# Rick0514/SimpleSLAM

Measured on AMD Instinct MI355X. Metric: scans/s (65 k-pt scan vs 1 M-pt submap, LOAM 10 iters) + pose RMSE vs CPU ref, higher is better.
Workload: dtype f64; 1 GPU; pcr=loam, 65536-pt 64-beam scan vs 1000000-pt submap, 10 GN iters, early exit off, index rebuilt per call (previous call's bounding box and tile layout reused as checked hints), inputs in HBM; parallelism=single GPU, scans_cycled=8

## Files before the change

### include/pcr_hip.h

```cpp
#ifndef PCR_HIP_H
#define PCR_HIP_H

#include <stddef.h>
#include <stdint.h>

#ifdef __cplusplus
extern "C" {
#endif

typedef struct pcr_handle pcr_handle;

typedef struct pcr_params {
    uint32_t struct_size;
    int32_t device;

    int32_t loam_iters;
    int32_t loam_early_exit;
    double loam_knn_max_sq;
    double loam_plane_thresh;
    double loam_point_thresh;
    double loam_pos_conv;
    double loam_rot_conv;

    double ndt_resolution;
// ... 19 lines not shown
    int32_t record_timeline;
    int32_t loam_coresident;
    int32_t loam_clamp_margin_mm;
    int32_t full_target;
    int32_t host_optimiser;
    int32_t host_copy_xyz;
} pcr_params;

typedef struct pcr_stats {
    double total_ms;
    double index_ms;
    double solve_ms;
    double kernel_ms;
    int32_t kernel_launches;
    int32_t iterations;
    int64_t n_src, n_dst;
    int32_t attempts;
    int32_t target_builds;
    int32_t region_repeats;
    int32_t region_index;
    double aux_kernel_ms;
    int64_t region_points, region_voxels, pairs_grad, pairs_hess;
    int32_t index_box_hint, index_layout_hint;
} pcr_stats;

void pcr_default_params(pcr_params* p);

pcr_handle* pcr_create(const char* method, const pcr_params* p);
void pcr_destroy(pcr_handle* h);
const char* pcr_last_error(const pcr_handle* h);

int pcr_scan2map(pcr_handle* h, const void* src, size_t n_src, const void* dst, size_t n_dst,
                 size_t stride_bytes, double pose_inout[16], int* converged);

int pcr_host_pin(const void* ptr, size_t bytes);
int pcr_host_unpin(const void* ptr);

int pcr_scan2map_device(pcr_handle* h, const void* d_src, size_t n_src, const void* d_dst, size_t n_dst,
                        size_t stride_bytes, double pose_inout[16], int* converged);

int pcr_set_target(pcr_handle* h, const void* dst, size_t n_dst, size_t stride_bytes, int on_device);
int pcr_align(pcr_handle* h, const void* src, size_t n_src, size_t stride_bytes, int on_device,
              double pose_inout[16], int* converged);
int pcr_invalidate_target(pcr_handle* h);

double pcr_fitness(pcr_handle* h);
// ... 166 lines not shown
```

### simpleslam_amd/csrc/capi.hip

```cpp
#include <dlfcn.h>
#include <math.h>
#include <string.h>

#include <algorithm>
#include <atomic>
#include <functional>
#include <mutex>
#include <vector>

#include "pcr_internal.h"
#include "ndt_opt.h"
#include "vgicp_opt.h"
#include "small_math.h"

using namespace pcr;

namespace {

thread_local std::string g_create_error;

enum Method { kLoam = 0, kNdt = 1, kVgicp = 2 };

struct NcclId { char internal[128]; };
typedef int (*nccl_get_id_fn)(NcclId*);
// ... 286 lines not shown
    a->c.knn_max_sq = h->prm.loam_knn_max_sq; a->c.plane_thresh = h->prm.loam_plane_thresh;
    a->c.point_thresh = h->prm.loam_point_thresh; a->c.pos_conv = h->prm.loam_pos_conv; a->c.rot_conv = h->prm.loam_rot_conv;
    a->c.iters = h->prm.loam_iters; a->c.early_exit = h->prm.loam_early_exit;
    memcpy(a->init_pose, pose, 16 * sizeof(double));
    a->state = h->loam_state.as<LoamState>();
    a->partials = h->loam_partials.as<double>();
    a->reduced = nullptr;
    a->n_partials = loam_grid_blocks((uint32_t)n_src);
    h->last_blocks = a->n_partials;
    a->trace = h->prm.record_trace ? h->loam_trace.as<LoamTrace>() : nullptr;
    a->result = h->result.dev;
    a->coresident = h->prm.loam_coresident == 1;
    if (h->prm.loam_disable_cache == 0 && h->nn_cache.reserve((n_src + 1) * 192) == hipSuccess) a->nn_cache = (NnCacheEntry*)h->nn_cache.p;
    if (h->prm.record_timeline == 1 && h->timeline.reserve((size_t)(std::max(1, h->prm.loam_iters) + 1) * kMaxPartials * kTimelineSlots * sizeof(unsigned long long)) == hipSuccess)
        a->timeline = h->timeline.as<unsigned long long>();
    a->use_tile = h->use_tile;
    for (int d = 0; d < 3; ++d) { a->tile_lo[d] = h->tile_lo[d]; a->tile_hi[d] = h->tile_hi[d]; }
}

int build_target(pcr_handle* h, const float* d_dst, size_t n_dst, size_t stride_floats) {
    double cell = 1.0;
    if (h->method == kLoam) cell = grid_cell_for(h->prm.loam_knn_max_sq);
    h->grid.no_hints = h->prm.index_no_hints != 0;
    hipError_t e = h->grid.build(d_dst, n_dst, stride_floats, cell, h->stream, &h->err, 0.0, 0, h->clamp.use ? &h->clamp : nullptr, h->method == kLoam);
    if (e != hipSuccess) return 1;
    h->tgt_ptr = d_dst; h->tgt_n = n_dst; h->tgt_stride = stride_floats; h->have_target = true;
    return 0;
}

static constexpr double kClampMargin = 10.0;
static constexpr int kClampRetries = 6;

int set_clamp_from_scan(pcr_handle* h, const float* d_src, size_t n_src, size_t stride_floats, const double pose[16]) {
    if (!n_src) return fail(h, "target bounding box too large for the dense index and the scan is empty");
    if (h->src_grid.build(d_src, n_src, stride_floats, 1.0, h->stream, &h->err) != hipSuccess) return 1;
    GridHeader sh;
    H_TRY(hipMemcpyAsync(&sh, h->src_grid.header.p, sizeof sh, hipMemcpyDeviceToHost, h->stream));
    H_TRY(hipStreamSynchronize(h->stream));
    if (sh.empty) return fail(h, "target bounding box too large for the dense index and the scan has no finite point");
    double lo[3], hi[3], mlo[3] = {1e300, 1e300, 1e300}, mhi[3] = {-1e300, -1e300, -1e300};
    for (int d = 0; d < 3; ++d) { lo[d] = sh.origin[d]; hi[d] = sh.origin[d] + sh.dims[d] * sh.cell; }
    for (int c = 0; c < 8; ++c) {
        const double p[3] = {c & 1 ? hi[0] : lo[0], c & 2 ? hi[1] : lo[1], c & 4 ? hi[2] : lo[2]};
        for (int r = 0; r < 3; ++r) {
            const double v = pose[r] * p[0] + pose[4 + r] * p[1] + pose[8 + r] * p[2] + pose[12 + r];
            mlo[r] = std::min(mlo[r], v); mhi[r] = std::max(mhi[r], v);
        }
// ... 32 lines not shown
    if (!overflow) return 0;
    if (need_cells > 4000000000ull && h->method == kLoam && d_src && pose && !h->clamp.use) {
        if (set_clamp_from_scan(h, d_src, n_src, stride_floats, pose)) return 1;
        if (build_target(h, h->tgt_ptr, h->tgt_n, h->tgt_stride)) return 1;
        return 2;
    }
    if (need_cells > 4000000000ull && h->method == kLoam && h->clamp_from_bulk && !h->clamp.use) {
        if (set_clamp_from_target_sample(h)) return 1;
        if (build_target(h, h->tgt_ptr, h->tgt_n, h->tgt_stride)) return 1;
        return 2;
    }
    if (h->grid.grow_cells(need_cells, &h->err) != hipSuccess) return 1;
    if (build_target(h, h->tgt_ptr, h->tgt_n, h->tgt_stride)) return 1;
    return 2;
}

int settle_loam_index(pcr_handle* h, const float* d_src, size_t n_src, size_t stride_floats, const double* pose) {
    for (int attempt = 0; attempt < 6; ++attempt) {
        GridHeader hdr;
        H_TRY(hipMemcpyAsync(&hdr, h->grid.header.p, sizeof(hdr), hipMemcpyDeviceToHost, h->stream));
        H_TRY(hipStreamSynchronize(h->stream));
        if (hdr.stale) {
            h->grid.hint_margin = 8; h->grid.cells_hint = 0;
            if (build_target(h, h->tgt_ptr, h->tgt_n, h->tgt_stride)) return 1;
            continue;
        }
        const int ov = check_grid_overflow(h, hdr.overflow, hdr.n_cells, h->clamp_allowed ? d_src : nullptr, n_src, stride_floats, pose);
        if (ov == 0) { if (!hdr.empty) { h->grid.confirm(); h->grid.note_cells(hdr.n_cells); } return 0; }
        if (ov == 1) return 1;
    }
    return fail(h, "target index could not be sized");
}

int run_loam(pcr_handle* h, const float* d_src, size_t n_src, size_t stride_floats, double pose[16], int* converged,
             bool index_timed) {
    if (n_src > 0xfffffff0ull) return fail(h, "source cloud too large");
    if (peer_check(h)) return 1;
    if (ensure_loam_buffers(h)) return 1;
    const int iters = std::max(0, h->prm.loam_iters);
    const bool shard = sharded(h);
    h->clamp_margin = h->prm.loam_clamp_margin_mm != 0 ? 1e-3 * h->prm.loam_clamp_margin_mm : kClampMargin;
    const double margin_cap = kClampMargin * (1 << kClampRetries);
    for (int attempt = 0; attempt < 24; ++attempt) {
        bool rank_fail = false;
        std::string rank_err;
        if (shard) {
// ... 57 lines not shown
            volatile int32_t* flag = &h->result.host->pad;
            for (int spin = 0; spin < 200000 && *flag != 1; ++spin) __builtin_ia32_pause();
            std::atomic_thread_fence(std::memory_order_acquire);
            if (*flag != 1) H_TRY(hipStreamSynchronize(h->stream));
        } else {
            H_TRY(hipStreamSynchronize(h->stream));
        }
        const LoamResult r = *h->result.host;
        if (r.pad != 1) return fail(h, "LOAM finalize kernel did not complete");
        if (peer_check(h)) return 1;
        if (r.fail == 2 || rank_fail)
            return fail(h, rank_fail ? "this rank could not index its map tile: " + rank_err : "sharded scan2map: another rank could not index its map tile");
        if (r.fail == 3) {
            h->clamp_margin = std::max(2.0 * h->clamp_margin, h->clamp_margin + 1.0);
            if (h->clamp_margin > margin_cap) return fail(h, "the pose left the region of a target too sparse for the dense index (a stray point far from the map?)");
            if (h->clamp.use) {
                if (set_clamp_from_scan(h, d_src, n_src, stride_floats, pose)) { if (!shard) return 1; h->grid.valid = false; }
                else if (build_target(h, h->tgt_ptr, h->tgt_n, h->tgt_stride)) { if (!shard) return 1; }
            }
            index_timed = false;
            continue;
        }
        if (!shard) {
            if (r.grid_stale) {
                h->grid.hint_margin = 8; h->grid.cells_hint = 0;
                if (build_target(h, h->tgt_ptr, h->tgt_n, h->tgt_stride)) return 1;
                index_timed = false;
                continue;
            }
            int ov = check_grid_overflow(h, r.grid_overflow, r.grid_cells, h->clamp_allowed ? d_src : nullptr, n_src, stride_floats, pose);
            if (ov == 1) return 1;
            if (ov == 2) { index_timed = false; continue; }
            if (!h->clamp.use && !r.grid_empty) { h->grid.confirm(); h->grid.note_cells(r.grid_cells); }
        }
        memcpy(pose, r.pose, 16 * sizeof(double));
        if (converged) *converged = r.converged;
        h->stats.iterations = r.iters_run; h->stats.attempts = attempt + 1;
        h->stats.n_src = (int64_t)n_src; h->stats.n_dst = (int64_t)h->tgt_n;
        h->stats.kernel_ms = 0; h->stats.kernel_launches = 0;
        if (h->profile >= 1 && read_call_times(h)) return 1;
        if (per_kernel) {
            const int used = std::min(iters, r.converged || r.fail ? r.iters_run : iters);
            for (int k = 0; k < used; ++k) {
                float ms = 0;
                H_TRY(hipEventElapsedTime(&ms, h->ev_kernel[2 * k], h->ev_kernel[2 * k + 1]));
                h->stats.kernel_ms += ms; h->stats.kernel_launches++;
// ... 1524 lines not shown

int pcr_get_timeline(pcr_handle* h, uint64_t* out, size_t capacity, int* launches, int* blocks) {
    if (!h) return 1;
    if (h->prm.record_timeline != 1 || !h->timeline.p) return fail(h, "timeline not recorded: set pcr_params.record_timeline = 1");
    const int nl = std::max(1, h->prm.loam_iters), nb = (int)h->last_blocks;
    if (launches) *launches = nl;
    if (blocks) *blocks = nb;
    if (!out) return 0;
    if (capacity < (size_t)nl * nb * kTimelineSlots) return fail(h, "timeline buffer too small");
    H_TRY(hipStreamSynchronize(h->stream));
    for (int l = 0; l < nl; ++l)
        H_TRY(hipMemcpy(out + (size_t)l * nb * kTimelineSlots, h->timeline.as<unsigned long long>() + (size_t)l * kMaxPartials * kTimelineSlots,
                        (size_t)nb * kTimelineSlots * sizeof(uint64_t),
                        hipMemcpyDeviceToHost));
    return 0;
}

int pcr_get_stats(pcr_handle* h, pcr_stats* out) {
    if (!h || !out) return 1;
    *out = h->stats;
    out->target_builds = (int32_t)h->target_builds;
    out->region_repeats = (int32_t)h->roi_repeats; out->region_index = (h->roi_on && h->grid.filtered) ? 1 : 0;
    out->index_box_hint = h->grid.used_hint ? 1 : 0; out->index_layout_hint = h->grid.used_layout ? 1 : 0;
    return 0;
}

int pcr_set_profile(pcr_handle* h, int level) {
    if (!h) return 1;
    h->profile = level < 0 ? 0 : (level > 2 ? 2 : level);
    return 0;
}

int pcr_set_stream(pcr_handle* h, void* hip_stream) {
    if (!h) return 1;
    if (h->stream) { (void)hipStreamSynchronize(h->stream); pin_forget_stream(h->stream); }
    if (h->own_stream && h->stream) (void)hipStreamDestroy(h->stream);
    h->stream = (hipStream_t)hip_stream;
    h->own_stream = false;
    return 0;
}

int pcr_set_query_tile(pcr_handle* h, const double lo[3], const double hi[3]) {
    if (!h) return 1;
    h->err.clear();
    if (!lo || !hi || lo[0] > hi[0]) { h->use_tile = 0; h->have_halo = false; return 0; }
    if (h->method != kLoam) return fail(h, "pcr_set_query_tile serves loam handles; ndt and vgicp tiles are set with pcr_set_shard (voxel-aligned bounds + halo)");
// ... 410 lines not shown
    if (fitness_batch_run(h, *fit_grid, d_src, n_src, stride_bytes / 4, refined.data(), nc, max_sq, 0, fs.data(), fn.data())) return 1;
    *any = false;
    for (size_t c = 0; c < nc; ++c) {
        cands[c]->n_in = fn[c];
        cands[c]->score = fs[c];
        if (fn[c] <= 0) continue;
        if (!*any || fn[c] > fn[*best] || (fn[c] == fn[*best] && fs[c] < fs[*best])) { *best = c; *any = true; }
    }
    return 0;
}

void reloc_point_fitness_at(pcr_handle* h, const double pose[16]) {
    if (h->fit_pending) { memcpy(h->fit_pose, pose, sizeof h->fit_pose); h->fitness = 1.7976931348623157e308; }
}

int query_index_for(pcr_handle* h, const char* who, size_t n_q, size_t stride_bytes, const GridIndex** grid) {
    if (!h->have_target || !h->grid.valid) return fail(h, std::string(who) + ": no kept target: call pcr_set_target first");
    if (batch_preconditions(h, n_q, stride_bytes)) { h->err = std::string(who) + ": " + h->err; return 1; }
    if (ensure_full_target(h)) return 1;
    if (fit_grid_for(h, grid)) return 1;
    GridHeader hdr;
    H_TRY(hipMemcpyAsync(&hdr, (*grid)->header.p, sizeof hdr, hipMemcpyDeviceToHost, h->stream));
    H_TRY(hipStreamSynchronize(h->stream));
    if (hdr.overflow || hdr.stale || (*grid)->filtered) return fail(h, std::string(who) + ": the target index is not complete (internal)");
    if (hdr.clamped)
        return fail(h, std::string(who) + ": the target's box cannot be tabulated and its index was cut to the bulk of the cloud: an exact query needs every point");
    return 0;
}

}

extern "C" {

int pcr_fitness_batch(pcr_handle* h, const void* src, size_t n_src, size_t stride_bytes, int on_device, const double* poses, size_t K,
                      double max_sq, size_t score_points, double* scores, int64_t* n_in) {
    if (!h) return 1;
    h->err.clear();
    if (K > PCR_RELOC_MAX_POSES) return fail(h, "K = " + std::to_string(K) + " is more than PCR_RELOC_MAX_POSES (" + std::to_string(PCR_RELOC_MAX_POSES) + ")");
    if (K && (!poses || !scores || !n_in)) return fail(h, "poses, scores or n_in is NULL");
    if (n_src && !src) return fail(h, "NULL cloud with nonzero size");
    if (batch_preconditions(h, n_src, stride_bytes)) return 1;
    const GridIndex* fit_grid = nullptr;
    if (fit_grid_for(h, &fit_grid)) return 1;
    if (K == 0) return 0;
    if (batch_points_check(h, n_src, score_points)) return 1;
    const float* d_src = (const float*)src;
    if (!on_device && stage_host(h, &h->src_stage, src, n_src, stride_bytes, &d_src)) return 1;
// ... 296 lines not shown
```

### simpleslam_amd/csrc/grid_index.hip

```cpp
#include "pcr_internal.h"
#include <stdlib.h>
#include <algorithm>
#include <string.h>

namespace pcr {

static constexpr int kScanPerThread = 8;
static constexpr int kScanBlock = 256;
static constexpr int kScanTile = kScanPerThread * kScanBlock;

__device__ inline float wave_min(float v) {
#pragma unroll
    for (int m = 32; m >= 1; m >>= 1) v = fminf(v, __shfl_xor(v, m, 64));
    return v;
}
__device__ inline float wave_max(float v) {
#pragma unroll
    for (int m = 32; m >= 1; m >>= 1) v = fmaxf(v, __shfl_xor(v, m, 64));
    return v;
}

__global__ __launch_bounds__(256) void grid_bbox_header_kernel(const float* __restrict__ pts, uint32_t n, uint32_t stride,
                                                               float* __restrict__ partials, uint32_t* __restrict__ ticket,
                                                               GridHeader* __restrict__ hdr, uint64_t capacity, double cell, double shift, int pcl_mode,
// ... 43 lines not shown
    for (uint32_t b = threadIdx.x; b < gridDim.x; b += 256) {
        float t[6];
#pragma unroll
        for (int d = 0; d < 6; ++d) t[d] = __hip_atomic_load(&partials[b * 6 + d], __ATOMIC_RELAXED, __HIP_MEMORY_SCOPE_AGENT);
#pragma unroll
        for (int d = 0; d < 3; ++d) { fmn[d] = fminf(fmn[d], t[d]); fmx[d] = fmaxf(fmx[d], t[3 + d]); }
    }
    __syncthreads();
#pragma unroll
    for (int d = 0; d < 3; ++d) {
        float a = wave_min(fmn[d]), b = wave_max(fmx[d]);
        if (lane == 0) { sh[wave][d] = a; sh[wave][3 + d] = b; }
    }
    __syncthreads();
    if (threadIdx.x == 0) *ticket = 0;
    if (threadIdx.x < 2 && (threadIdx.x == 0 || twin.hdr)) {
        const bool second = threadIdx.x == 1;
        if (second) { cell = twin.cell; capacity = twin.capacity; hdr = twin.hdr; mirror = twin.mirror; }
        GridHeader h;
        h.cell = cell; h.inv_cell = 1.0 / cell; h.n_points = n; h.shift = shift;
        h.empty = 0; h.overflow = 0;
        h.pcl_mode = pcl_mode; h.inv_leaf_f = 1.0f / (float)cell; h.too_fine = 0; h.sum_sq = 0.f; h.sum_sq_u = 0ull;
        h.min_b[0] = h.min_b[1] = h.min_b[2] = 0;
        h.clamped = (clamp.use && !pcl_mode) ? 1 : 0; h.cut_mask = 0; h.stale = 0; h.pad2_ = 0;
        double nc = 1.0, nc_tight = 1.0;
        int mg_xy = margin_xy, mg_z = margin_z_pcl;
        if (pcl_mode) {
            double padded = 1.0;
            for (int d = 0; d < 3; ++d) {
                const float lo = fminf(fminf(sh[0][d], sh[1][d]), fminf(sh[2][d], sh[3][d]));
                const float hi = fmaxf(fmaxf(sh[0][3 + d], sh[1][3 + d]), fmaxf(sh[2][3 + d], sh[3][3 + d]));
                if (!(lo <= hi)) continue;
                nc_tight *= (double)truncf((hi - lo) * h.inv_leaf_f) + 1.0;
                padded *= (double)floorf(hi * h.inv_leaf_f) - (double)floorf(lo * h.inv_leaf_f) + 1.0 + 2.0 * (d < 2 ? mg_xy : mg_z);
            }
            if (padded > 4.0e9) mg_xy = mg_z = 0;
        }
        for (int d = 0; d < 3; ++d) {
            float lo = fminf(fminf(sh[0][d], sh[1][d]), fminf(sh[2][d], sh[3][d]));
            float hi = fmaxf(fmaxf(sh[0][3 + d], sh[1][3 + d]), fmaxf(sh[2][3 + d], sh[3][3 + d]));
            if (!(lo <= hi)) { h.empty = 1; lo = hi = 0.f; }
            if (h.clamped) {
                if (lo < (float)clamp.lo[d]) h.cut_mask |= 1 << d;
                if (hi > (float)clamp.hi[d]) h.cut_mask |= 8 << d;
                lo = fmaxf(lo, (float)clamp.lo[d]); hi = fminf(hi, (float)clamp.hi[d]);
                if (!(lo <= hi)) { h.empty = 1; lo = hi = 0.f; }
            }
// ... 231 lines not shown
    else { const float* p = pts + i * stride; x = p[0]; y = p[1]; z = p[2]; }
}

template <bool kVec, int kBinPer, bool kPlace, bool kSub, bool kPacked = false>
__global__ __launch_bounds__(256) void grid_bin_kernel(const float* __restrict__ pts, uint32_t n_in, uint32_t stride, GridHeader* __restrict__ hdr,
                                                       uint32_t* __restrict__ bin_count, uint32_t* __restrict__ slot, int shift, uint32_t max_tiles, uint32_t nb_max,
                                                       uint32_t* __restrict__ ticket, uint32_t* __restrict__ bin_start,
                                                       const uint32_t* __restrict__ lay_cur, float4* __restrict__ tiled, uint32_t tiled_cap,
                                                       const uint8_t* __restrict__ keep_mask, int keep_mshift, uint32_t* __restrict__ n_packed = nullptr) {
    static_assert(!kPacked || (kVec && kPlace), "a packed list is float4 and is placed by a layout");
    static_assert(kPlace || !kSub, "tiles are cut by a layout only");
    extern __shared__ __attribute__((aligned(16))) uint32_t dyn_lds[];
    uint32_t* const hist = dyn_lds;
    uint32_t* const sh_lay = dyn_lds + nb_max;
    uint16_t* const sh_sub = reinterpret_cast<uint16_t*>(dyn_lds + 2 * (size_t)nb_max + 2);
    constexpr uint32_t kBinChunk = 256u * kBinPer;
    const uint32_t c_first = blockIdx.x * kBinChunk;
    uint32_t nb_lay = 0, nt_lay = 0;
    if (kPlace) { nb_lay = lay_cur[kLayMeta]; nt_lay = lay_cur[kLayMeta + 1]; }
    uint32_t n = n_in;
    if (kPacked) n = min(*n_packed, n_in);
    const GridHeader h = *hdr;
    if (h.overflow || h.empty) { if (kPacked && blockIdx.x == 0 && threadIdx.x == 0) *n_packed = 0u; return; }
    const uint32_t ntiles = (uint32_t)(h.n_cells >> shift) + 1u;
    const uint32_t nb = kPlace ? nb_lay : ntiles;
    if (kPlace) {
        if (nb == 0u || nb > nb_max || nt_lay != ntiles || ntiles > max_tiles || (!kSub && nb != ntiles)) { if (threadIdx.x == 0) hdr->stale = 3; return; }
        for (uint32_t b = threadIdx.x; b <= nb; b += 256) sh_lay[b] = lay_cur[b];
        if (kSub) for (uint32_t t = threadIdx.x; t < ntiles; t += 256) sh_sub[t] = (uint16_t)lay_cur[kLaySub + t];
    }
    for (uint32_t b = threadIdx.x; b < nb_max; b += 256) hist[b] = 0u;
    __syncthreads();
    const int lane = threadIdx.x & 63;
    for (uint32_t c0 = c_first; c0 < n; c0 += gridDim.x * kBinChunk) {
        uint32_t bin[kBinPer], loc[kBinPer];
        bool first[kBinPer];
        float px[kBinPer], py[kBinPer], pz[kBinPer];
        uint32_t pw[kPacked ? kBinPer : 1];
#pragma unroll
        for (int u = 0; u < kBinPer; ++u) {
            const uint32_t i = c0 + u * 256 + threadIdx.x;
            if (kPacked) { const float4 v = reinterpret_cast<const float4*>(pts)[i < n ? i : c0]; px[u] = v.x; py[u] = v.y; pz[u] = v.z; pw[u] = __float_as_uint(v.w); }
            else load_xyz<kVec>(pts, i < n ? i : c0, stride, px[u], py[u], pz[u]);
        }
#pragma unroll
        for (int u = 0; u < kBinPer; ++u) {
// ... 114 lines not shown
            uint32_t key, cc[3];
            bool out_u = false;
            mi[u] = 0xffffffffu;
            if (i < n && point_key(h, px[u], py[u], pz[u], &key, &out_u, cc)) mi[u] = roi_macro(h, mshift, (int)cc[0], (int)cc[1], (int)cc[2]);
            outside = outside || (i < n && out_u);
        }
        if (outside && !h.clamped) hdr->stale = 1;
        uint8_t mb[kPer];
#pragma unroll
        for (int u = 0; u < kPer; ++u) mb[u] = mask[mi[u] != 0xffffffffu ? mi[u] : 0u];
        uint32_t mine = 0;
#pragma unroll
        for (int u = 0; u < kPer; ++u) { mb[u] = (mi[u] != 0xffffffffu && mb[u] != 0) ? 1 : 0; mine += mb[u]; }
        uint32_t total;
        uint32_t off = block_exclusive_scan_256(mine, &total, sh4);
        if (threadIdx.x == 0) sh_base = total ? atomicAdd(counter, total) : 0u;
        __syncthreads();
        off += sh_base;
#pragma unroll
        for (int u = 0; u < kPer; ++u)
            if (mb[u]) { if (off < out_cap) out[off] = make_float4(px[u], py[u], pz[u], __uint_as_float(c0 + u * 256 + threadIdx.x)); ++off; }
        __syncthreads();
    }
}

template <bool kVec>
__global__ __launch_bounds__(256) void grid_place_kernel(const float* __restrict__ pts, uint32_t n, uint32_t stride, const GridHeader* __restrict__ hdr,
                                                         const uint32_t* __restrict__ bin_count, const uint32_t* __restrict__ slot,
                                                         const uint32_t* __restrict__ bin_start, float4* __restrict__ tiled, int shift) {
    extern __shared__ __attribute__((aligned(16))) uint32_t dyn_lds[];
    uint32_t* const sh_start = dyn_lds;
    const GridHeader h = *hdr;
    if (h.overflow || h.empty) return;
    const uint32_t nbins = (uint32_t)(h.n_cells >> shift) + 1u;
    constexpr int kPer = 4;
    float px[kPer], py[kPer], pz[kPer];
    uint32_t sl[kPer];
    uint32_t c0 = blockIdx.x * (256 * kPer);
#pragma unroll
    for (int u = 0; u < kPer; ++u) {
        const uint32_t i = c0 + u * 256 + threadIdx.x;
        load_xyz<kVec>(pts, i < n ? i : 0u, stride, px[u], py[u], pz[u]);
        sl[u] = i < n ? slot[i] : 0xffffffffu;
    }
    for (uint32_t b = threadIdx.x; b <= nbins; b += 256) sh_start[b] = bin_start[b];
    __syncthreads();
// ... 429 lines not shown
#pragma unroll
        for (int k = 0; k < 2 * kRoiMaxRadius + 3; ++k) any |= w[k];
        out[m] = any ? 1 : 0;
    }
}

hipError_t roi_launch(const GridIndex& lattice, const float* d_src, size_t n_src, size_t stride_floats, const Pose16& T, int mshift,
                      uint8_t* d_mark, uint8_t* d_mark_next, uint8_t* d_tmp, uint8_t* d_mask, double base_m, double per_m, hipStream_t s, const BlobStore* blob) {
    const int mb = (int)std::min<size_t>(1024, (n_src + 255) / 256 ? (n_src + 255) / 256 : 1);
    static BlobStore no_blob;
    hipLaunchKernelGGL(roi_mark_kernel, dim3(mb), dim3(256), 0, s, d_src, (uint32_t)n_src, (uint32_t)stride_floats, T, lattice.header.as<GridHeader>(), d_mark, mshift, base_m, per_m,
                       blob ? *blob : no_blob);
    const size_t macros = (lattice.cell_capacity >> (3 * mshift)) + 1024;
    const int db = (int)std::min<size_t>(4096, (macros + 255) / 256);
    const GridHeader* hdr = lattice.header.as<GridHeader>();
    hipLaunchKernelGGL(roi_spread_axis_kernel, dim3(db), dim3(256), 0, s, hdr, (const uint8_t*)d_mark, d_tmp, d_mark_next, 1, mshift, T.m[12], T.m[13], T.m[14], base_m, per_m);
    hipLaunchKernelGGL(roi_spread_axis_kernel, dim3(db), dim3(256), 0, s, hdr, (const uint8_t*)d_tmp, d_mask, (uint8_t*)nullptr, 2, mshift, T.m[12], T.m[13], T.m[14], base_m, per_m);
    return hipGetLastError();
}

hipError_t GridIndex::enqueue_density(hipStream_t s) {
    if (tiled_shift < 0) return hipSuccess;
    hipLaunchKernelGGL(grid_density_kernel, dim3(1), dim3(256), 0, s, header.as<GridHeader>(), tile_sq.as<unsigned long long>(), tiled_shift,
                       used_layout ? (const uint32_t*)layout[lay_idx ^ 1].as<uint32_t>() : (const uint32_t*)nullptr);
    return hipGetLastError();
}

hipError_t DeviceBuf::reserve(size_t bytes) {
    if (bytes <= cap) return hipSuccess;
    release();
    size_t want = 2 * bytes + 256;
    hipError_t e = hipMalloc(&p, want);
    if (e != hipSuccess) { p = nullptr; cap = 0; return e; }
    cap = want;
    return hipSuccess;
}
void DeviceBuf::release() {
    if (p) (void)hipFree(p);
    p = nullptr; cap = 0;
}

void GridIndex::release() {
    sorted.release(); cell_count.release(); cell_start.release(); block_sums.release();
    bbox_partials.release(); header.release(); keys.release(); ranks.release(); ticket.release();
    tiled.release(); bin_count.release(); bin_start.release(); tile_sq.release(); kept.release(); layout[0].release(); layout[1].release(); lay_ok = false;
    cell_capacity = 0; valid = false; n_points = 0;
}
// ... 22 lines not shown
}

#define PCR_TRY(x) do { hipError_t _e = (x); if (_e != hipSuccess) { if (err) *err = std::string(#x) + ": " + hipGetErrorString(_e); return _e; } } while (0)

hipError_t GridIndex::ensure_tables(hipStream_t s, std::string* err) {
    PCR_TRY(header.reserve(sizeof(GridHeader)));
    if (cell_capacity == 0) {
        size_t guess = 1u << 20;
        PCR_TRY(cell_count.reserve((guess + kScanTile) * sizeof(uint32_t)));
        PCR_TRY(cell_start.reserve((guess + kScanTile) * sizeof(uint32_t)));
        PCR_TRY(hipMemsetAsync(cell_count.p, 0, cell_count.cap, s));
        cell_capacity = guess;
        PCR_TRY(block_sums.reserve(2 * (guess / kScanTile + 2) * sizeof(uint32_t)));
    }
    return hipSuccess;
}
size_t GridIndex::effective_capacity() const {
    size_t cap_eff = cell_capacity;
    if (cells_hint) cap_eff = std::min<size_t>(cell_capacity, std::max<size_t>(2 * (size_t)cells_hint + 64, 1024));
    return cap_eff;
}

hipError_t GridIndex::build(const float* d_pts, size_t n, size_t stride_floats, double cell, hipStream_t s, std::string* err, double shift,
                            int pcl_mode, const ClampBox* clamp, bool allow_hint, BuildFilter* filter) {
    valid = false;
    filtered = false;
    if (filter) { filter->applied = false; filter->tail_applied = false; }
    if (n > 0xfffffff0ull) { if (err) *err = "target cloud too large (>= 2^32 points)"; return hipErrorInvalidValue; }
    const size_t n_res = std::max(n, reserve_points);
    PCR_TRY(sorted.reserve((n_res + 16) * sizeof(float4)));
    PCR_TRY(bbox_partials.reserve(kBBoxBlocks * 6 * sizeof(float)));
    PCR_TRY(keys.reserve((n_res + 1) * sizeof(uint32_t)));
    PCR_TRY(ranks.reserve((n_res + 1) * sizeof(uint32_t)));
    if (!ticket.p) {
        PCR_TRY(ticket.reserve(256));
        PCR_TRY(hipMemsetAsync(ticket.p, 0, 256, s));
    }
    PCR_TRY(ensure_tables(s, err));
    ClampBox cb;
    memset(&cb, 0, sizeof cb);
    if (clamp) cb = *clamp;
    const uint32_t n32 = (uint32_t)n, st = (uint32_t)stride_floats;
    const int pt_blocks = (int)std::min<size_t>(2048, (n + 255) / 256 ? (n + 255) / 256 : 1);
    const size_t cap_eff = effective_capacity();
    const size_t tiles_target = std::min<size_t>(4096, std::max<size_t>(64, n / 512));
    int tshift;
    const int tshift_cap = cut_sparse ? 12 : 11;
    if (cells_hint) { tshift = 2; while ((cells_hint >> tshift) > tiles_target && tshift < tshift_cap) ++tshift; }
    else { tshift = 8; while (((uint64_t)cap_eff >> tshift) + 2 > 2048 && tshift < 11) ++tshift; }
// ... 27 lines not shown
        tiled_shift = tshift;
        if (!bin_count.p) {
            PCR_TRY(bin_count.reserve(((size_t)kMaxBins + 64) * kBinStride * sizeof(uint32_t)));
            PCR_TRY(hipMemsetAsync(bin_count.p, 0, bin_count.cap, s));
        }
        const bool vec = (stride_floats % 4 == 0) && ((uintptr_t)d_pts % 16 == 0);
        const size_t bin_chunk = (size_t)256 * kBinPerThread;
        const int bin_blocks = (int)std::min<size_t>(4096, (n + bin_chunk - 1) / bin_chunk ? (n + bin_chunk - 1) / bin_chunk : 1);
        const int place_blocks = (int)std::min<size_t>(2048, (n + 1023) / 1024 ? (n + 1023) / 1024 : 1);
        const bool sparse = split_sparse_tiles && cells_hint > 4 * (uint64_t)n + 65536;
        const uint64_t tiles_est = cells_hint ? (cells_hint >> tshift) + 1 : 0;
        const bool per8 = !sparse && tiles_est && n / tiles_est <= 1024;
        const uint32_t hs = per8 ? 2048u : (sparse && cut_sparse ? 3072u : 0xffffffffu);
        uint32_t nb_max = (uint32_t)std::min<uint64_t>((uint64_t)kMaxBins, std::max<uint64_t>((uint64_t)max_bins, (tiles_est ? tiles_est + 2 : (uint64_t)max_bins) + (hs != 0xffffffffu ? 2 * (uint64_t)n / hs : 0)));
        if (hs == 0xffffffffu && !(lay_ok && lay_cuts)) nb_max = max_bins;
        if (lay_ok && lay_shift == tshift) nb_max = std::max(nb_max, lay_nb_max);
        const bool use_layout = reuse_header && lay_ok && lay_shift == tshift && lay_nb_max <= nb_max;
        for (int i = 0; i < 2; ++i)
            if (!layout[i].p) { PCR_TRY(layout[i].reserve(kLayWords * sizeof(uint32_t))); PCR_TRY(hipMemsetAsync(layout[i].p, 0, kLayWords * sizeof(uint32_t), s)); }
        if (use_layout) {
            const size_t need = 2 * (lay_n + (lay_n >> lay_room_shift)) + (size_t)lay_room_add * (nb_max + 1) + 16;
            if (need > n + 16) PCR_TRY(tiled.reserve(need * sizeof(float4)));
        }
        const uint32_t tiled_cap = (uint32_t)std::min<size_t>(tiled.cap / sizeof(float4), 0xfffffff0u);
        const uint32_t* const lay_cur = layout[lay_idx].as<uint32_t>();
        uint32_t* const lay_next = layout[lay_idx ^ 1].as<uint32_t>();
        used_layout = use_layout;
        const uint8_t* keep_mask = nullptr;
        int keep_mshift = 0;
        if (filter && use_layout && filter->enqueue_mask) {
            PCR_TRY(filter->enqueue_mask());
            keep_mask = filter->mask; keep_mshift = filter->mshift;
            filter->applied = filtered = keep_mask != nullptr;
        }
        const bool cuts_now = hs != 0xffffffffu;
        const bool use_sub = use_layout && lay_cuts;
        const bool plan_lds = cuts_now || use_sub;
        const uint32_t nb_bin = use_layout ? nb_max : max_bins;
        const size_t bin_lds = (size_t)nb_bin * 4 + (use_layout ? ((size_t)nb_bin + 4) * 4 : 0) + (use_sub ? ((size_t)max_bins + 8) * 2 : 0), place_lds = ((size_t)max_bins + 4) * 4,
                     tile_lds = std::max<size_t>((size_t)(1u << tshift) * 4, plan_lds ? ((size_t)nb_max + 4) * 4 + ((size_t)max_bins + 8) * 2 : 0);
#define PCR_LAUNCH_BIN(VEC, PER, PLACE, SUB) hipLaunchKernelGGL((grid_bin_kernel<VEC, PER, PLACE, SUB>), dim3(bin_blocks), dim3(256), bin_lds, s, d_pts, n32, st, header.as<GridHeader>(), \
                                                    bin_count.as<uint32_t>(), ranks.as<uint32_t>(), tshift, max_bins, nb_bin, ticket.as<uint32_t>() + 8, bin_start.as<uint32_t>(), \
                                                    lay_cur, tiled.as<float4>(), tiled_cap, keep_mask, keep_mshift)
#define PCR_LAUNCH_BIN_P(VEC, PLACE, SUB) PCR_LAUNCH_BIN(VEC, kBinPerThread, PLACE, SUB)
        const bool keep_pass = keep_mask != nullptr && n >= 2000000;
        if (keep_pass) {
// ... 30 lines not shown
        plan.lay_next = lay_next; plan.hs = hs; plan.nb_max = nb_max; plan.enabled = 1; plan.copy_only = filtered ? 1 : 0; plan.cuts = cuts_now ? 1 : 0; plan.room_shift = lay_room_shift; plan.room_add = lay_room_add; plan.pad_ = 0;
        const uint32_t bins_bound = use_layout ? nb_max : max_bins;
        const uint32_t bins_expected = tiles_est ? (uint32_t)std::min<uint64_t>(bins_bound, tiles_est + 16 + (use_layout && hs != 0xffffffffu ? (uint64_t)n / hs : 0)) : bins_bound;
        const int tile_blocks = (int)bins_expected + 1;
#define PCR_LAUNCH_TILE_R(PER, MODE, THREADS, TAIL, PLAN, RUNS) hipLaunchKernelGGL((grid_tile_kernel<PER, MODE, THREADS, TAIL, PLAN, RUNS>), dim3(tile_blocks), dim3(THREADS), (PLAN) ? tile_lds : (size_t)(1u << tshift) * 4, s, header.as<GridHeader>(), tile_sq.as<unsigned long long>(), \
                           bin_start.as<uint32_t>(), bin_count.as<uint32_t>(), tiled.as<float4>(), cell_start.as<uint32_t>(), sorted.as<float4>(), keys.as<uint32_t>(), tshift, \
                           use_layout ? lay_cur : (const uint32_t*)bin_start.as<uint32_t>(), use_layout ? lay_cur : (const uint32_t*)nullptr, plan, tail)
#define PCR_LAUNCH_TILE_T(PER, MODE, THREADS, TAIL, PLAN) PCR_LAUNCH_TILE_R(PER, MODE, THREADS, TAIL, PLAN, false)
#define PCR_LAUNCH_TILE(PER, MODE, THREADS) PCR_LAUNCH_TILE_T(PER, MODE, THREADS, false, true)
        const bool with_tail = filtered && filter->want_tail && !sparse && tshift <= 13;
        if (with_tail) { tail = filter->tail; tail.mask = keep_mask; tail.mshift = keep_mshift; filter->tail_applied = true; }
        if (coherent_input && sparse) { PCR_LAUNCH_TILE_R(1, 1, 256, false, false, true); PCR_LAUNCH_TILE_R(4, 2, 1024, false, true, true); }
        else if (coherent_input && !with_tail) { if (per8) PCR_LAUNCH_TILE_R(8, 0, 256, false, true, true); else PCR_LAUNCH_TILE_R(16, 0, 256, false, true, true); }
        else if (sparse) { PCR_LAUNCH_TILE_T(1, 1, 256, false, false); PCR_LAUNCH_TILE(16, 2, 256); }
        else if (with_tail) { if (per8) PCR_LAUNCH_TILE_T(8, 0, 256, true, true); else PCR_LAUNCH_TILE_T(16, 0, 256, true, true); }
        else if (per8) PCR_LAUNCH_TILE(8, 0, 256);
        else PCR_LAUNCH_TILE(16, 0, 256);
#undef PCR_LAUNCH_TILE
#undef PCR_LAUNCH_TILE_T
#undef PCR_LAUNCH_TILE_R
        lay_nb_max = nb_max; lay_cuts = cuts_now || use_sub;
        lay_idx ^= 1; lay_ok = true; lay_shift = tshift;
        if (!filtered) lay_n = n;
        PCR_TRY(hipGetLastError());
        n_points = n;
        valid = true;
        return hipSuccess;
    }
    tiled_shift = -1;
    hipLaunchKernelGGL(grid_count_kernel, dim3(pt_blocks), dim3(256), 0, s, d_pts, n32, st, header.as<GridHeader>(),
                       cell_count.as<uint32_t>(), keys.as<uint32_t>(), ranks.as<uint32_t>());
    const int scan_blocks = (int)((cell_capacity + kScanTile - 1) / kScanTile);
    hipLaunchKernelGGL(grid_scan_local_kernel, dim3(scan_blocks), dim3(kScanBlock), 0, s, cell_count.as<uint32_t>(),
                       cell_start.as<uint32_t>(), block_sums.as<uint32_t>(), header.as<GridHeader>());
    hipLaunchKernelGGL(grid_scan_add_kernel, dim3(scan_blocks), dim3(kScanBlock), 0, s, cell_start.as<uint32_t>(),
                       block_sums.as<uint32_t>(), header.as<GridHeader>());
    hipLaunchKernelGGL(grid_scatter_kernel, dim3(pt_blocks), dim3(256), 0, s, d_pts, n32, st, header.as<GridHeader>(),
                       keys.as<uint32_t>(), ranks.as<uint32_t>(), cell_start.as<uint32_t>(), sorted.as<float4>());
    PCR_TRY(hipGetLastError());
    n_points = n;
    valid = true;
    return hipSuccess;
}

}
```

### simpleslam_amd/csrc/loam.hip

```cpp
#include <hip/hip_ext.h>

#include "pcr_internal.h"
#include "peer_exchange.h"
#include "small_math.h"

namespace pcr {



static constexpr int kNb = 8;
static constexpr uint32_t kNoPos = 0xffffffffu;
static constexpr uint32_t kKeyEmpty = 0xffffffffu;

struct Nb8 {
    double d[kNb];
    uint32_t idx[kNb];
    float x[kNb], y[kNb], z[kNb];
};

__device__ __forceinline__ bool knn_less(double d, uint32_t i, double d2, uint32_t i2) {
    return (d < d2) | ((d == d2) & (i < i2));
}

__device__ __forceinline__ double sqdist(double qx, double qy, double qz, float px, float py, float pz) {
// ... 942 lines not shown
#pragma unroll
        for (int c = 1; c < 8; ++c) v += sh_sum[c * 32 + tid];
        if (tid == 28) v = (double)(sh_cnt[0] + sh_cnt[2] + sh_cnt[4] + sh_cnt[6]);
        if (tid == 29) v = (double)(sh_cnt[1] + sh_cnt[3] + sh_cnt[5] + sh_cnt[7]);
        if (tid == kSlotEscapes) v = (double)(sh_cnt[8] + sh_cnt[9] + sh_cnt[10] + sh_cnt[11]);
        a.partials[((size_t)(k & 1) * kMaxPartials + blockIdx.x) * kAccum + tid] = v;
    }
    if (tl) tl[6] = wall_clock64();
}

__global__ __launch_bounds__(256) void loam_finalize_kernel(const LoamArgs a, const int k) {
    __shared__ double sh_sum[8 * 32];
    __shared__ Prologue sh_pro;
    loam_prologue(a, k, sh_sum, &sh_pro);
    if (threadIdx.x == 0) {
        double T[16];
        for (int i = 0; i < 16; ++i) T[i] = sh_pro.pose[i];
        t2se3(T);
        const LoamState* cur = &a.state[k & 1];
        LoamResult* r = a.result;
        for (int i = 0; i < 16; ++i) r->pose[i] = T[i];
        r->converged = cur->converged; r->iters_run = cur->iters_run; r->fail = cur->fail;
        r->grid_overflow = a.grid.hdr->overflow; r->grid_empty = a.grid.hdr->empty; r->grid_cells = a.grid.hdr->n_cells;
        r->grid_stale = a.grid.hdr->stale;
        __threadfence_system();
        __hip_atomic_store(&r->pad, 1, __ATOMIC_RELEASE, __HIP_MEMORY_SCOPE_SYSTEM);
    }
}

__device__ __forceinline__ double loam_fold_own_rows(const LoamArgs& a, int k, int comp, int slice) {
    const int done = a.state[k & 1].done;
    const double* const part0 = a.partials + (size_t)(k & 1) * kMaxPartials * kAccum + comp;
    const uint32_t last = a.n_partials ? a.n_partials - 1u : 0u;
    double pv[32];
#pragma unroll
    for (int u = 0; u < 32; ++u) { const uint32_t b = (uint32_t)slice + 8u * u; pv[u] = part0[(size_t)(b < last ? b : last) * kAccum]; }
    double acc = 0.0;
#pragma unroll
    for (int u = 0; u < 32; ++u) acc += ((uint32_t)slice + 8u * u < a.n_partials) ? pv[u] : 0.0;
    for (uint32_t b = (uint32_t)slice + 256u; b < a.n_partials; b += 8u) acc += part0[(size_t)b * kAccum];
    return done ? 0.0 : acc;
}

__global__ __launch_bounds__(256) void loam_reduce_kernel(const LoamArgs a, const int k, double* __restrict__ out) {
    __shared__ double sh_sum[8 * 32];
    const int t = threadIdx.x, comp = t & 31, slice = t >> 5;
    const double acc = loam_fold_own_rows(a, k, comp, slice);
// ... 69 lines not shown
```

### simpleslam_amd/csrc/pcr_internal.h

```cpp
#pragma once
#include <hip/hip_runtime.h>
#include <hip/hip_ext.h>
#include <stdint.h>
#include <functional>
#include <string>
#include <vector>

#include <stdlib.h>

#include "../../include/pcr_hip.h"

namespace pcr {

struct GridHeader {
    double origin[3];
    double org[3];
    double cell;
    double inv_cell;
    int32_t dims[3];
    uint32_t n_points;
    uint64_t n_cells;
    int32_t overflow;
    int32_t empty;
    double shift;
    int32_t pcl_mode;
    float inv_leaf_f;
    int32_t min_b[3];
    int32_t too_fine;
    float sum_sq;
    int32_t clamped;
    int32_t cut_mask;
    unsigned long long sum_sq_u;
    int32_t stale;
    int32_t pad2_;
};
__host__ __device__ inline double grid_sum_sq(const GridHeader& h) { return h.sum_sq_u ? (double)h.sum_sq_u : (double)h.sum_sq; }

struct ClampBox { double lo[3], hi[3]; int32_t use, pad_; };

struct HeaderTwin { GridHeader* hdr; GridHeader* mirror; uint64_t capacity; double cell; };

struct GridView {
    const GridHeader* hdr;
    const float4* pts;
    const uint32_t* cell_start;
};

static constexpr int kPad = 2;
static constexpr double kProgressWindow = 1048576.0;
static constexpr int kBBoxBlocks = 256;

struct Pose16 { double m[16]; };

struct LoamState {
    double pose[16];
    int32_t done;
    int32_t converged;
    int32_t iters_run;
    int32_t fail;
};

static constexpr int kAccum = 32;
static constexpr int kSlotRankFail = 30;
static constexpr int kSlotEscapes = 31;
static constexpr int kMaxPartials = 512;
static constexpr int kTimelineSlots = 16;

struct LoamConsts {
    double knn_max_sq, plane_thresh, point_thresh, pos_conv, rot_conv;
    int32_t iters, early_exit;
// ... 76 lines not shown
    DeviceBuf sorted, cell_count, cell_start, block_sums, bbox_partials, header, keys, ranks, ticket;
    DeviceBuf kept;
    DeviceBuf tiled, bin_count, bin_start, tile_sq;
    int tiled_shift = -1;
    bool hint_ok = false;
    double hint_cell = 0.0, hint_shift = 0.0;
    int hint_pcl = 0;
    int hint_margin = 0;
    int hint_margin_z_pcl = 0;
    bool used_hint = false;
    bool no_hints = false;
    bool coherent_input = false;
    bool cut_sparse = false;
    bool split_sparse_tiles = true;
    bool prefer_one_level = false;
    DeviceBuf layout[2];
    int lay_idx = 0, lay_shift = -1;
    uint32_t lay_nb_max = 0;
    bool lay_cuts = false;
    size_t lay_n = 0;
    uint32_t lay_room_add = 32;
    int lay_room_shift = 3;
    bool lay_ok = false, used_layout = false;
    bool filtered = false;
    GridHeader* header_mirror = nullptr;
    bool mirrored = false;
    GridIndex* twin = nullptr;
    double twin_cell = 0.0;
    bool header_preset = false;
    const float* preset_pts = nullptr; size_t preset_n = 0; double preset_cell = 0.0;
    hipError_t ensure_tables(hipStream_t s, std::string* err);
    size_t effective_capacity() const;
    void confirm() { hint_ok = valid && tiled_shift >= 0; }
    size_t cell_capacity = 0;
    uint64_t cells_hint = 0;
    void note_cells(uint64_t n_cells) { if (n_cells) cells_hint = n_cells; }
    size_t n_points = 0;
    size_t reserve_points = 0;
    bool valid = false;
    GridView view() const {
        return GridView{header.as<GridHeader>(), sorted.as<float4>(), cell_start.as<uint32_t>()};
    }
    hipError_t build(const float* d_pts, size_t n, size_t stride_floats, double cell, hipStream_t s,
                     std::string* err, double shift = 0.0, int pcl_mode = 0, const ClampBox* clamp = nullptr, bool allow_hint = false,
                     BuildFilter* filter = nullptr);
    hipError_t grow_cells(uint64_t need_cells, std::string* err);
    hipError_t enqueue_density(hipStream_t s);
    void release();
};

struct VgicpVoxel {
    double mean[3];
    double cov[6];
    double w;
    uint32_t n, pad;
};

struct RoiView {
    const GridHeader* lat;
    const uint8_t* mask;
    uint32_t* escapes;
    int32_t mshift;
    int32_t filtered;
    uint32_t* count;
};
__host__ __device__ inline uint32_t roi_macro(const GridHeader& h, int mshift, int cx, int cy, int cz) {
    const uint32_t m0 = ((uint32_t)h.dims[0] + (1u << mshift) - 1u) >> mshift, m1 = ((uint32_t)h.dims[1] + (1u << mshift) - 1u) >> mshift;
    return (((uint32_t)cz >> mshift) * m1 + ((uint32_t)cy >> mshift)) * m0 + ((uint32_t)cx >> mshift);
// ... 141 lines not shown
```

### simpleslam_amd/pcr.py

```python
import ctypes as C
import os

import numpy as np

_HERE = os.path.dirname(os.path.abspath(__file__))
LIB_PATH = os.environ.get("PCR_LIB") or os.path.join(_HERE, "lib", "libpcr_hip.so")


class PcrParams(C.Structure):
    _fields_ = [
        ("struct_size", C.c_uint32), ("device", C.c_int32),
        ("loam_iters", C.c_int32), ("loam_early_exit", C.c_int32),
        ("loam_knn_max_sq", C.c_double), ("loam_plane_thresh", C.c_double), ("loam_point_thresh", C.c_double),
        ("loam_pos_conv", C.c_double), ("loam_rot_conv", C.c_double),
        ("ndt_resolution", C.c_double), ("ndt_step_size", C.c_double), ("ndt_outlier_ratio", C.c_double),
        ("ndt_trans_eps", C.c_double), ("ndt_max_iters", C.c_int32), ("ndt_min_points", C.c_int32),
        ("vgicp_resolution", C.c_double), ("vgicp_k_corr", C.c_int32), ("vgicp_max_iters", C.c_int32),
        ("vgicp_lm_inner", C.c_int32), ("vgicp_rot_eps", C.c_double), ("vgicp_trans_eps", C.c_double),
        ("vgicp_lm_init_scale", C.c_double),
        ("record_trace", C.c_int32),
        ("index_no_hints", C.c_int32), ("ndt_evaluate_repeats", C.c_int32), ("loam_disable_cache", C.c_int32), ("record_timeline", C.c_int32),
        ("loam_coresident", C.c_int32), ("loam_clamp_margin_mm", C.c_int32), ("full_target", C.c_int32), ("host_optimiser", C.c_int32),
        ("host_copy_xyz", C.c_int32),
    ]


class PcrStats(C.Structure):
    _fields_ = [
        ("total_ms", C.c_double), ("index_ms", C.c_double), ("solve_ms", C.c_double), ("kernel_ms", C.c_double),
        ("kernel_launches", C.c_int32), ("iterations", C.c_int32), ("n_src", C.c_int64), ("n_dst", C.c_int64),
        ("attempts", C.c_int32), ("target_builds", C.c_int32), ("region_repeats", C.c_int32), ("region_index", C.c_int32),
        ("aux_kernel_ms", C.c_double), ("region_points", C.c_int64), ("region_voxels", C.c_int64), ("pairs_grad", C.c_int64), ("pairs_hess", C.c_int64),
        ("index_box_hint", C.c_int32), ("index_layout_hint", C.c_int32),
    ]


ABI_SYMBOLS = [
    "pcr_default_params", "pcr_create", "pcr_destroy", "pcr_last_error", "pcr_scan2map", "pcr_scan2map_device", "pcr_host_pin", "pcr_host_unpin",
    "pcr_set_target", "pcr_align", "pcr_invalidate_target", "pcr_fitness", "pcr_loam_linearize", "pcr_get_trace", "pcr_get_trace_counts",
    "pcr_vgicp_covariances", "pcr_vgicp_neighbours", "pcr_vgicp_linearize", "pcr_voxel_filter", "pcr_voxel_filter_begin", "pcr_voxel_filter_end", "pcr_get_timeline", "pcr_ndt_derivatives", "pcr_get_stats", "pcr_set_profile", "pcr_set_stream", "pcr_set_query_tile", "pcr_comm_unique_id", "pcr_comm_init", "pcr_comm_info", "pcr_comm_peer_export", "pcr_comm_init_peer",
    "pcr_comm_init_host", "pcr_set_shard", "pcr_set_params", "pcr_get_params", "pcr_fitness_gated",
    "pcr_map_create", "pcr_map_destroy", "pcr_map_last_error", "pcr_map_add_keyframe", "pcr_map_keyframes", "pcr_map_clear", "pcr_map_update", "pcr_map_update_begin", "pcr_map_wait", "pcr_map_update_window", "pcr_map_submap",
    "pcr_map_submap_indices", "pcr_map_generation", "pcr_scan2map_submap",
    "pcr_ndt_opt_create", "pcr_ndt_opt_destroy", "pcr_ndt_opt_request", "pcr_ndt_opt_feed", "pcr_ndt_opt_result", "pcr_ndt_opt_counts",
    "pcr_vgicp_opt_create", "pcr_vgicp_opt_destroy", "pcr_vgicp_opt_request", "pcr_vgicp_opt_feed", "pcr_vgicp_opt_result",
    "pcr_sc_default_params", "pcr_sc_create", "pcr_sc_destroy", "pcr_sc_last_error", "pcr_sc_size", "pcr_sc_add", "pcr_sc_descriptor", "pcr_sc_distance",
    "pcr_sc_query", "pcr_knn", "pcr_radius_search", "pcr_fitness_batch", "pcr_reloc_default_params", "pcr_reloc_hypotheses", "pcr_relocalize",
    "pcr_sc_distances", "pcr_global_reloc_default_params", "pcr_global_reloc_hypotheses", "pcr_relocalize_global",
]

ALLREDUCE_FN = C.CFUNCTYPE(C.c_int, C.POINTER(C.c_double), C.c_size_t, C.c_int, C.c_void_p)


class ScParams(C.Structure):
    _fields_ = [("lidar_height", C.c_double), ("num_exclude_recent", C.c_int32), ("build_tree_gap", C.c_int32), ("num_candidates", C.c_int32),
                ("pad", C.c_int32), ("search_ratio", C.c_double), ("dist_thres", C.c_double)]
# ... 786 lines not shown
```

Before: 3933 scans/s.

## Replay previous target index permutation with per-point cell verification

When the target has the same point count and stride as the last successful LOAM build, the sort/scatter index build is skipped. A replay kernel instead reloads each point at its previous sorted slot and checks that it still falls within its cell's range in the existing cell_start table. Any mismatch sets a replay_miss flag. The host then rebuilds the index in full and backs off exponentially before trying replay again. This trades the full counting-sort rebuild for one gather-and-verify pass, at the cost of an extra rebuild whenever the map changes.

```diff
diff --git a/include/pcr_hip.h b/include/pcr_hip.h
--- a/include/pcr_hip.h
+++ b/include/pcr_hip.h
@@ -65,6 +65,7 @@
     double aux_kernel_ms;
     int64_t region_points, region_voxels, pairs_grad, pairs_hess;
     int32_t index_box_hint, index_layout_hint;
+    int32_t index_replayed, index_replay_misses, index_replay_skip, index_replay_wait;
 } pcr_stats;
 
 void pcr_default_params(pcr_params* p);
diff --git a/simpleslam_amd/csrc/capi.hip b/simpleslam_amd/csrc/capi.hip
--- a/simpleslam_amd/csrc/capi.hip
+++ b/simpleslam_amd/csrc/capi.hip
@@ -332,7 +332,8 @@
     double cell = 1.0;
     if (h->method == kLoam) cell = grid_cell_for(h->prm.loam_knn_max_sq);
     h->grid.no_hints = h->prm.index_no_hints != 0;
-    hipError_t e = h->grid.build(d_dst, n_dst, stride_floats, cell, h->stream, &h->err, 0.0, 0, h->clamp.use ? &h->clamp : nullptr, h->method == kLoam);
+    hipError_t e = h->grid.build(d_dst, n_dst, stride_floats, cell, h->stream, &h->err, 0.0, 0, h->clamp.use ? &h->clamp : nullptr, h->method == kLoam, nullptr,
+                                 h->method == kLoam && !sharded(h));
     if (e != hipSuccess) return 1;
     h->tgt_ptr = d_dst; h->tgt_n = n_dst; h->tgt_stride = stride_floats; h->have_target = true;
     return 0;
@@ -411,6 +412,11 @@
         H_TRY(hipStreamSynchronize(h->stream));
         if (hdr.stale) {
             h->grid.hint_margin = 8; h->grid.cells_hint = 0;
+            if (build_target(h, h->tgt_ptr, h->tgt_n, h->tgt_stride)) return 1;
+            continue;
+        }
+        if (hdr.replay_miss) {
+            h->grid.replay_missed();
             if (build_target(h, h->tgt_ptr, h->tgt_n, h->tgt_stride)) return 1;
             continue;
         }
@@ -514,6 +520,12 @@
             continue;
         }
         if (!shard) {
+            if (r.grid_stale == kGridReplayMiss) {
+                h->grid.replay_missed();
+                if (build_target(h, h->tgt_ptr, h->tgt_n, h->tgt_stride)) return 1;
+                index_timed = false;
+                continue;
+            }
             if (r.grid_stale) {
                 h->grid.hint_margin = 8; h->grid.cells_hint = 0;
                 if (build_target(h, h->tgt_ptr, h->tgt_n, h->tgt_stride)) return 1;
@@ -2084,6 +2096,8 @@
     out->target_builds = (int32_t)h->target_builds;
     out->region_repeats = (int32_t)h->roi_repeats; out->region_index = (h->roi_on && h->grid.filtered) ? 1 : 0;
     out->index_box_hint = h->grid.used_hint ? 1 : 0; out->index_layout_hint = h->grid.used_layout ? 1 : 0;
+    out->index_replayed = h->grid.replayed ? 1 : 0; out->index_replay_misses = (int32_t)h->grid.rp_misses;
+    out->index_replay_skip = (int32_t)h->grid.rp_skip; out->index_replay_wait = (int32_t)h->grid.rp_wait;
     return 0;
 }
 
@@ -2540,7 +2554,7 @@
     GridHeader hdr;
     H_TRY(hipMemcpyAsync(&hdr, (*grid)->header.p, sizeof hdr, hipMemcpyDeviceToHost, h->stream));
     H_TRY(hipStreamSynchronize(h->stream));
-    if (hdr.overflow || hdr.stale || (*grid)->filtered) return fail(h, std::string(who) + ": the target index is not complete (internal)");
+    if (hdr.overflow || hdr.stale || hdr.replay_miss || (*grid)->filtered) return fail(h, std::string(who) + ": the target index is not complete (internal)");
     if (hdr.clamped)
         return fail(h, std::string(who) + ": the target's box cannot be tabulated and its index was cut to the bulk of the cloud: an exact query needs every point");
     return 0;
diff --git a/simpleslam_amd/csrc/grid_index.hip b/simpleslam_amd/csrc/grid_index.hip
--- a/simpleslam_amd/csrc/grid_index.hip
+++ b/simpleslam_amd/csrc/grid_index.hip
@@ -89,7 +89,7 @@
         h.empty = 0; h.overflow = 0;
         h.pcl_mode = pcl_mode; h.inv_leaf_f = 1.0f / (float)cell; h.too_fine = 0; h.sum_sq = 0.f; h.sum_sq_u = 0ull;
         h.min_b[0] = h.min_b[1] = h.min_b[2] = 0;
-        h.clamped = (clamp.use && !pcl_mode) ? 1 : 0; h.cut_mask = 0; h.stale = 0; h.pad2_ = 0;
+        h.clamped = (clamp.use && !pcl_mode) ? 1 : 0; h.cut_mask = 0; h.stale = 0; h.replay_miss = 0;
         double nc = 1.0, nc_tight = 1.0;
         int mg_xy = margin_xy, mg_z = margin_z_pcl;
         if (pcl_mode) {
@@ -367,6 +367,7 @@
     if (kPacked) n = min(*n_packed, n_in);
     const GridHeader h = *hdr;
     if (h.overflow || h.empty) { if (kPacked && blockIdx.x == 0 && threadIdx.x == 0) *n_packed = 0u; return; }
+    if (blockIdx.x == 0 && threadIdx.x == 0 && h.n_points != n_in) hdr->n_points = n_in;
     const uint32_t ntiles = (uint32_t)(h.n_cells >> shift) + 1u;
     const uint32_t nb = kPlace ? nb_lay : ntiles;
     if (kPlace) {
@@ -527,6 +528,47 @@
             if (mb[u]) { if (off < out_cap) out[off] = make_float4(px[u], py[u], pz[u], __uint_as_float(c0 + u * 256 + threadIdx.x)); ++off; }
         __syncthreads();
     }
+}
+
+template <bool kVec>
+__global__ __launch_bounds__(256) void grid_replay_kernel(const float* __restrict__ pts, uint32_t n, uint32_t stride, GridHeader* __restrict__ hdr,
+                                                          const uint32_t* __restrict__ cell_start, float4* sorted) {
+    constexpr int kPer = 4;
+    const GridHeader h = *hdr;
+    if (h.overflow || h.empty || h.stale || h.pcl_mode || h.n_points != n || n == 0u) {
+        if (threadIdx.x == 0) hdr->replay_miss = 1;
+        return;
+    }
+    bool miss = false;
+    for (uint32_t c0 = blockIdx.x * (256u * kPer); c0 < n; c0 += gridDim.x * (256u * kPer)) {
+        uint32_t w[kPer], key[kPer], lo[kPer], hi[kPer];
+        float px[kPer], py[kPer], pz[kPer];
+        bool ok[kPer];
+#pragma unroll
+        for (int u = 0; u < kPer; ++u) {
+            const uint32_t j = c0 + u * 256 + threadIdx.x;
+            w[u] = __float_as_uint(sorted[j < n ? j : n - 1u].w);
+        }
+#pragma unroll
+        for (int u = 0; u < kPer; ++u) load_xyz<kVec>(pts, w[u] < n ? w[u] : n - 1u, stride, px[u], py[u], pz[u]);
+#pragma unroll
+        for (int u = 0; u < kPer; ++u) {
+            key[u] = 0u;
+            ok[u] = w[u] < n && point_key(h, px[u], py[u], pz[u], &key[u]);
+            if (!ok[u]) key[u] = 0u;
+        }
+#pragma unroll
+        for (int u = 0; u < kPer; ++u) { lo[u] = cell_start[key[u]]; hi[u] = cell_start[key[u] + 1u]; }
+#pragma unroll
+        for (int u = 0; u < kPer; ++u) {
+            const uint32_t j = c0 + u * 256 + threadIdx.x;
+            if (j < n) {
+                if (ok[u] && lo[u] <= j && j < hi[u]) sorted[j] = make_float4(px[u], py[u], pz[u], __uint_as_float(w[u]));
+                else miss = true;
+            }
+        }
+    }
+    if (miss) hdr->replay_miss = 1;
 }
 
 template <bool kVec>
@@ -1002,7 +1044,7 @@
 hipError_t GridIndex::enqueue_density(hipStream_t s) {
     if (tiled_shift < 0) return hipSuccess;
     hipLaunchKernelGGL(grid_density_kernel, dim3(1), dim3(256), 0, s, header.as<GridHeader>(), tile_sq.as<unsigned long long>(), tiled_shift,
-                       used_layout ? (const uint32_t*)layout[lay_idx ^ 1].as<uint32_t>() : (const uint32_t*)nullptr);
+                       dens_by_layout ? (const uint32_t*)layout[lay_idx ^ 1].as<uint32_t>() : (const uint32_t*)nullptr);
     return hipGetLastError();
 }
 
@@ -1071,9 +1113,11 @@
 }
 
 hipError_t GridIndex::build(const float* d_pts, size_t n, size_t stride_floats, double cell, hipStream_t s, std::string* err, double shift,
-                            int pcl_mode, const ClampBox* clamp, bool allow_hint, BuildFilter* filter) {
+                            int pcl_mode, const ClampBox* clamp, bool allow_hint, BuildFilter* filter, bool allow_replay) {
     valid = false;
     filtered = false;
+    const bool rp_armed = rp_ok;
+    rp_ok = rp_full = replayed = false;
     if (filter) { filter->applied = false; filter->tail_applied = false; }
     if (n > 0xfffffff0ull) { if (err) *err = "target cloud too large (>= 2^32 points)"; return hipErrorInvalidValue; }
     const size_t n_res = std::max(n, reserve_points);
@@ -1147,6 +1191,20 @@
             const size_t need = 2 * (lay_n + (lay_n >> lay_room_shift)) + (size_t)lay_room_add * (nb_max + 1) + 16;
             if (need > n + 16) PCR_TRY(tiled.reserve(need * sizeof(float4)));
         }
+        bool replay = allow_replay && use_layout && rp_armed && pcl_mode == 0 && !filter && n > 0 && rp_n == n && rp_stride == stride_floats;
+        if (replay && rp_wait) { --rp_wait; replay = false; }
+        if (replay) {
+            used_layout = true;
+            const bool vec4 = (stride_floats % 4 == 0) && ((uintptr_t)d_pts % 16 == 0);
+            const int blocks = (int)std::min<size_t>(4096, (n + 1023) / 1024);
+            if (vec4) hipLaunchKernelGGL(grid_replay_kernel<true>, dim3(blocks), dim3(256), 0, s, d_pts, n32, st, header.as<GridHeader>(), (const uint32_t*)cell_start.as<uint32_t>(), sorted.as<float4>());
+            else hipLaunchKernelGGL(grid_replay_kernel<false>, dim3(blocks), dim3(256), 0, s, d_pts, n32, st, header.as<GridHeader>(), (const uint32_t*)cell_start.as<uint32_t>(), sorted.as<float4>());
+            PCR_TRY(hipGetLastError());
+            replayed = true; rp_full = true;
+            n_points = n;
+            valid = true;
+            return hipSuccess;
+        }
         const uint32_t tiled_cap = (uint32_t)std::min<size_t>(tiled.cap / sizeof(float4), 0xfffffff0u);
         const uint32_t* const lay_cur = layout[lay_idx].as<uint32_t>();
         uint32_t* const lay_next = layout[lay_idx ^ 1].as<uint32_t>();
@@ -1223,6 +1281,8 @@
         lay_nb_max = nb_max; lay_cuts = cuts_now || use_sub;
         lay_idx ^= 1; lay_ok = true; lay_shift = tshift;
         if (!filtered) lay_n = n;
+        dens_by_layout = use_layout;
+        rp_full = !filtered && !cb.use; rp_n = n; rp_stride = stride_floats;
         PCR_TRY(hipGetLastError());
         n_points = n;
         valid = true;
diff --git a/simpleslam_amd/csrc/loam.hip b/simpleslam_amd/csrc/loam.hip
--- a/simpleslam_amd/csrc/loam.hip
+++ b/simpleslam_amd/csrc/loam.hip
@@ -988,7 +988,7 @@
         for (int i = 0; i < 16; ++i) r->pose[i] = T[i];
         r->converged = cur->converged; r->iters_run = cur->iters_run; r->fail = cur->fail;
         r->grid_overflow = a.grid.hdr->overflow; r->grid_empty = a.grid.hdr->empty; r->grid_cells = a.grid.hdr->n_cells;
-        r->grid_stale = a.grid.hdr->stale;
+        r->grid_stale = a.grid.hdr->stale ? a.grid.hdr->stale : (a.grid.hdr->replay_miss ? kGridReplayMiss : 0);
         __threadfence_system();
         __hip_atomic_store(&r->pad, 1, __ATOMIC_RELEASE, __HIP_MEMORY_SCOPE_SYSTEM);
     }
diff --git a/simpleslam_amd/csrc/pcr_internal.h b/simpleslam_amd/csrc/pcr_internal.h
--- a/simpleslam_amd/csrc/pcr_internal.h
+++ b/simpleslam_amd/csrc/pcr_internal.h
@@ -2,6 +2,7 @@
 #include <hip/hip_runtime.h>
 #include <hip/hip_ext.h>
 #include <stdint.h>
+#include <algorithm>
 #include <functional>
 #include <string>
 #include <vector>
@@ -32,7 +33,7 @@
     int32_t cut_mask;
     unsigned long long sum_sq_u;
     int32_t stale;
-    int32_t pad2_;
+    int32_t replay_miss;
 };
 __host__ __device__ inline double grid_sum_sq(const GridHeader& h) { return h.sum_sq_u ? (double)h.sum_sq_u : (double)h.sum_sq; }
 
@@ -46,6 +47,7 @@
     const uint32_t* cell_start;
 };
 
+static constexpr int32_t kGridReplayMiss = 0x100;
 static constexpr int kPad = 2;
 static constexpr double kProgressWindow = 1048576.0;
 static constexpr int kBBoxBlocks = 256;
@@ -168,6 +170,14 @@
     uint32_t lay_room_add = 32;
     int lay_room_shift = 3;
     bool lay_ok = false, used_layout = false;
+    bool dens_by_layout = false;
+    bool rp_full = false;
+    bool rp_ok = false;
+    size_t rp_n = 0, rp_stride = 0;
+    bool replayed = false;
+    uint32_t rp_misses = 0;
+    uint32_t rp_skip = 0, rp_wait = 0;
+    void replay_missed() { rp_misses += 1; rp_skip = rp_skip ? std::min<uint32_t>(64u, 2u * rp_skip) : 1u; rp_wait = rp_skip; rp_ok = rp_full = false; hint_ok = false; }
     bool filtered = false;
     GridHeader* header_mirror = nullptr;
     bool mirrored = false;
@@ -177,7 +187,11 @@
     const float* preset_pts = nullptr; size_t preset_n = 0; double preset_cell = 0.0;
     hipError_t ensure_tables(hipStream_t s, std::string* err);
     size_t effective_capacity() const;
-    void confirm() { hint_ok = valid && tiled_shift >= 0; }
+    void confirm() {
+        hint_ok = valid && tiled_shift >= 0;
+        rp_ok = hint_ok && rp_full;
+        if (rp_ok && replayed) rp_skip = rp_wait = 0;
+    }
     size_t cell_capacity = 0;
     uint64_t cells_hint = 0;
     void note_cells(uint64_t n_cells) { if (n_cells) cells_hint = n_cells; }
@@ -189,7 +203,7 @@
     }
     hipError_t build(const float* d_pts, size_t n, size_t stride_floats, double cell, hipStream_t s,
                      std::string* err, double shift = 0.0, int pcl_mode = 0, const ClampBox* clamp = nullptr, bool allow_hint = false,
-                     BuildFilter* filter = nullptr);
+                     BuildFilter* filter = nullptr, bool allow_replay = false);
     hipError_t grow_cells(uint64_t need_cells, std::string* err);
     hipError_t enqueue_density(hipStream_t s);
     void release();
diff --git a/simpleslam_amd/pcr.py b/simpleslam_amd/pcr.py
--- a/simpleslam_amd/pcr.py
+++ b/simpleslam_amd/pcr.py
@@ -32,6 +32,7 @@
         ("attempts", C.c_int32), ("target_builds", C.c_int32), ("region_repeats", C.c_int32), ("region_index", C.c_int32),
         ("aux_kernel_ms", C.c_double), ("region_points", C.c_int64), ("region_voxels", C.c_int64), ("pairs_grad", C.c_int64), ("pairs_hess", C.c_int64),
         ("index_box_hint", C.c_int32), ("index_layout_hint", C.c_int32),
+        ("index_replayed", C.c_int32), ("index_replay_misses", C.c_int32), ("index_replay_skip", C.c_int32), ("index_replay_wait", C.c_int32),
     ]
 
 
```

Result: faster. 4380 scans/s (median of 6 runs) (+11.4%).
